# Sir-Teo/MuZero-Go

Hardware: AMD Instinct MI355X
Metric: MCTS simulations/sec (whole node) + self-play moves/sec, 9x9 Go, 200 sims/move (higher is better)
Workload: dtype fp32

## Files before the change

include/mzgo.h:

```cpp
#ifndef MZGO_H
#define MZGO_H

#include <stdint.h>

#ifdef __cplusplus
extern "C" {
#endif

enum {
  MZGO_OK = 0,
  MZGO_EINVAL = -1,
  MZGO_EHIP = -2,
  MZGO_ENOWEIGHTS = -3,
  MZGO_EASSERT = -4
};

typedef struct mzgo_config {
  int board_size;
  int latent_dim;
  int num_games;
  int num_simulations;
  int max_moves;
  int compat;
  int temperature_moves;
  int search_variant;
  double c_puct;
  double discount;
  double dirichlet_alpha;
  double dirichlet_epsilon;
  double pass_epsilon;
  double temperature;
  double komi;
  uint64_t seed;
  int game_base;
  int device;
  int direct_dynamics;
  int tower;
  int res_blocks;
  int fast_simulations;
  double full_search_prob;
} mzgo_config;

typedef struct mzgo_engine mzgo_engine;

void mzgo_default_config(mzgo_config* cfg, int board_size);

int mzgo_engine_create(const mzgo_config* cfg, mzgo_engine** out);
void mzgo_engine_destroy(mzgo_engine* eng);
int mzgo_playout_budget_host(uint64_t seed, uint32_t key_gid, int move, int num_simulations, int fast_simulations,
                             double full_search_prob, int* budget);
const char* mzgo_last_error(void);
int64_t mzgo_engine_device_bytes(const mzgo_engine* eng);

int mzgo_set_weights(mzgo_engine* eng, const char* key, const float* data_host,
                     const int64_t* shape, int ndim);
int mzgo_weights_ready(const mzgo_engine* eng);

int mzgo_set_weights_device(mzgo_engine* eng, const char* const* keys, const float* const* data_dev,
                            const int64_t* const* shapes, const int* ndims, int n, void* stream);
int mzgo_weights_copy(mzgo_engine* dst, const mzgo_engine* src, void* stream);
int mzgo_weights_export(mzgo_engine* eng, float* data_host, int64_t cap, int64_t* n_floats, void* stream);
int mzgo_weights_pack_host(int board_size, int latent_dim, const char* const* keys, const float* const* data_host,
                           const int64_t* const* shapes, const int* ndims, int n, float* blob, int64_t cap,
                           int64_t* n_floats);

int mzgo_initial_inference(mzgo_engine* eng, const float* obs, int B, float* latent,
                           float* value, float* logits, void* stream);
int mzgo_recurrent_inference(mzgo_engine* eng, const float* latent, const int64_t* action, int B,
                             float* next_latent, float* reward, float* value, float* logits,
                             void* stream);
int mzgo_check_inference_errors(mzgo_engine* eng, void* stream);

int mzgo_search(mzgo_engine* eng, const float* root_obs, const double* noise, int G, int move_index,
                int32_t* root_child_visits, double* root_value, void* stream);
int mzgo_reanalyse(mzgo_engine* eng, const int8_t* stones, const uint8_t* invd, const uint8_t* flags,
                   const int32_t* ids, const double* noise, int n, int32_t* visits, double* value,
                   double* policy, void* stream);
int mzgo_tree_export(mzgo_engine* eng, int g, int32_t* n_nodes_host, int32_t* child_host,
                     int32_t* visits_host, double* value_sum_host, float* prior_host,
                     double* root_prior_host, void* stream);

int mzgo_board_reset(mzgo_engine* eng, void* stream);
int mzgo_board_step(mzgo_engine* eng, const int32_t* actions, int32_t* status, double* winner,
                    void* stream);
int mzgo_board_planes(mzgo_engine* eng, double* planes, void* stream);
int mzgo_board_set(mzgo_engine* eng, int g, const int8_t* stones_host, const uint8_t* invd_host,
                   const int32_t* meta_host, void* stream);

int mzgo_selfplay_reset(mzgo_engine* eng, int epoch, void* stream);
int mzgo_selfplay_move(mzgo_engine* eng, void* stream);
int mzgo_selfplay_moves(mzgo_engine* eng, int moves, void* stream);

int mzgo_arena_move(mzgo_engine* eng, mzgo_engine* opponent, void* stream);
int mzgo_arena_moves(mzgo_engine* eng, mzgo_engine* opponent, int moves, void* stream);
int mzgo_selfplay_counters(mzgo_engine* eng, uint64_t* counters_host, void* stream);
int mzgo_search_stats(mzgo_engine* eng, uint64_t* stats_host, void* stream);
int mzgo_search_stats2(mzgo_engine* eng, uint64_t* stats_host, int cap, void* stream);

int mzgo_selfplay_set_timing(mzgo_engine* eng, int on);
int mzgo_selfplay_launch_times(mzgo_engine* eng, float* boards_ms, float* queue_ms, int cap, int* n_host);
int mzgo_stream_wait_started(mzgo_engine* eng, uint64_t target, void* stream);
int mzgo_tower_timing(mzgo_engine* eng, int enable, double* tower_ms_host, int64_t* towers_host);

int mzgo_dyn_conv_backward_workspace(int B, int C, int64_t* bytes_host);
int mzgo_dyn_conv_backward(const float* grad_out, const float* out, const float* latent, const int64_t* action,
                           const float* emb, const float* weight, int B, int C, int N, float* grad_latent,
                           float* grad_weight, float* grad_bias, void* workspace, int64_t workspace_bytes,
                           void* stream);
int mzgo_conv3x3_relu_forward(const float* x, const int64_t* action, const float* emb, const float* weight,
                              const float* bias, int B, int Cin, int Cout, int N, float* out, void* stream);
int mzgo_conv3x3_backward_workspace(int B, int Cin, int Cout, int64_t* bytes_host);
int mzgo_conv3x3_backward(const float* grad_out, const float* out, const float* x, const int64_t* action,
                          const float* emb, const float* weight, int B, int Cin, int Cout, int N, float* grad_x,
                          float* grad_weight, float* grad_bias, void* workspace, int64_t workspace_bytes,
                          void* stream);
int mzgo_selfplay_inject_noise(mzgo_engine* eng, const double* noise);
int mzgo_selfplay_record_noise(mzgo_engine* eng, double* dst);
// ... 199 lines not shown
```

muzero-go_amd/csrc/mzgo_board.hpp:

```cpp
#pragma once
#include "mzgo_common.hpp"

namespace mzgo {

struct BoardMeta {
  int turn;
  int passed;
  int done;
  int moves;
};

template <class G>
struct BoardLds {
  int8_t* stone;
  uint8_t* invd;
  int* label;
  int* libs;
  int* gsize;
  int* killed;
  int* misc;
};

template <class G>
struct BoardWG {
  static constexpr int SIZE = G::THREADS;
  __device__ static int id() { return tid_local(); }
  __device__ static void sync() { __syncthreads(); }
  __device__ static bool any(int v) { return __syncthreads_or(v) != 0; }
  __device__ static bool leader() { return tid_local() == 0; }
};
template <class G>
__device__ __forceinline__ bool nbr(int c, int d, int& n) {
  const int r = c / G::N, col = c - r * G::N;
  switch (d) {
    case 0: if (r == 0) return false; n = c - G::N; return true;
    case 1: if (r == G::N - 1) return false; n = c + G::N; return true;
    case 2: if (col == 0) return false; n = c - 1; return true;
    default: if (col == G::N - 1) return false; n = c + 1; return true;
  }
}

template <class G, class T, class ClassFn>
__device__ __forceinline__ void label_components(int* label, ClassFn cls) {
  for (int c = T::id(); c < G::CELLS; c += T::SIZE) label[c] = cls(c) ? c : -1;
  T::sync();
  for (int it = 0; it < G::CELLS + 2; ++it) {
    int changed = 0;
    for (int c = T::id(); c < G::CELLS; c += T::SIZE) {
      const int k = cls(c);
      if (!k) continue;
      int m = label[c];
#pragma unroll
      for (int d = 0; d < 4; ++d) {
// ... 9 lines not shown
}

template <class G, class T>
__device__ __forceinline__ void count_liberties(BoardLds<G>& b, bool sizes) {
  for (int c = T::id(); c < G::CELLS; c += T::SIZE) { b.libs[c] = 0; if (sizes) b.gsize[c] = 0; }
  T::sync();
  for (int c = T::id(); c < G::CELLS; c += T::SIZE) {
    if (b.stone[c]) {
      if (sizes) atomicAdd(&b.gsize[b.label[c]], 1);
      continue;
    }
    int seen[4];
    int ns = 0;
#pragma unroll
    for (int d = 0; d < 4; ++d) {
      int n;
      if (nbr<G>(c, d, n) && b.stone[n]) {
        int l = b.label[n];
        bool dup = false;
        for (int i = 0; i < ns; ++i) dup |= seen[i] == l;
        if (!dup) { seen[ns++] = l; atomicAdd(&b.libs[l], 1); }
      }
    }
  }
  T::sync();
}

template <class G, class T>
__device__ __forceinline__ void compute_invalid(BoardLds<G>& b, int mover, int ko) {
  for (int c = T::id(); c < G::CELLS; c += T::SIZE) {
    uint8_t inv;
    if (b.stone[c]) {
      inv = 1;
    } else {
      bool boxed = true, maybe_bad = false, surely_ok = false;
#pragma unroll
      for (int d = 0; d < 4; ++d) {
        int n;
        if (!nbr<G>(c, d, n)) continue;
        const int s = b.stone[n];
        if (!s) { boxed = false; continue; }
        const int lib = b.libs[b.label[n]];
        if (s - 1 == mover) { maybe_bad |= lib > 1; surely_ok |= lib == 1; }
        else                { maybe_bad |= lib == 1; surely_ok |= lib > 1; }
      }
      inv = (boxed && maybe_bad && !surely_ok) ? 1 : 0;
    }
    b.invd[c] = inv;
  }
  T::sync();
  if (ko >= 0 && T::leader()) b.invd[ko] = 1;
  T::sync();
}

enum : int { BOARD_OK = 0, BOARD_ERR_DONE = 1, BOARD_ERR_INVALID = 2, BOARD_ERR_RANGE = 3 };

template <class G, class T = BoardWG<G>>
__device__ __forceinline__ int board_step(BoardLds<G>& b, BoardMeta& m, int action) {
  if (m.done) return BOARD_ERR_DONE;
  if (action < 0 || action > G::CELLS) return BOARD_ERR_RANGE;
  const int player = m.turn;
  int ko = -1;
  if (action == G::CELLS) {
    if (m.passed) m.done = 1;
    m.passed = 1;
    label_components<G, T>(b.label, [&](int c) { return (int)b.stone[c]; });
    count_liberties<G, T>(b, false);
  } else {
    if (b.invd[action]) return BOARD_ERR_INVALID;
    m.passed = 0;
    if (T::leader()) {
      b.stone[action] = (int8_t)(player + 1);
      bool boxed = true;
      for (int d = 0; d < 4; ++d) {
        int n;
        if (nbr<G>(action, d, n)) boxed &= b.stone[n] == 2 - player;
      }
      b.misc[1] = boxed;
    }
    T::sync();
    label_components<G, T>(b.label, [&](int c) { return (int)b.stone[c]; });
    count_liberties<G, T>(b, true);
    if (T::leader()) {
      int nk = 0;
      for (int d = 0; d < 4; ++d) {
        int n;
        if (!nbr<G>(action, d, n) || b.stone[n] != 2 - player) continue;
        const int l = b.label[n];
        bool dup = false;
        for (int i = 0; i < nk; ++i) dup |= b.killed[i] == l;
        if (!dup && b.libs[l] == 0) b.killed[nk++] = l;
      }
      b.misc[0] = nk;
      b.misc[2] = (nk == 1 && b.misc[1] && b.gsize[b.killed[0]] == 1) ? b.killed[0] : -1;
    }
    T::sync();
    const int nk = b.misc[0];
    ko = b.misc[2];
    if (nk > 0) {
      for (int c = T::id(); c < G::CELLS; c += T::SIZE) {
        if (b.stone[c] == 2 - player) {
          const int l = b.label[c];
          bool dead = false;
          for (int i = 0; i < nk; ++i) dead |= b.killed[i] == l;
          if (dead) b.stone[c] = 0;
        }
      }
      T::sync();
// ... 47 lines not shown
```

muzero-go_amd/csrc/mzgo_kernels.hpp:

```cpp
#pragma once
#include "mzgo_jobs.hpp"
#include "mzgo_replay.hpp"

namespace mzgo {

template <class G>
constexpr bool rep_needs_scratch() {
  if constexpr (G::WINO) return Wino<G>::NSTRIP > 1;
  else return false;
}

struct NoRepJobs {
  __device__ bool operator()(int) const { return false; }
};

template <class G, class PlaneFn, class Jobs = NoRepJobs>
__device__ __forceinline__ void representation(Smem<G>& sm, const NetParams& np, PlaneFn planes, float* lat,
                                      int lat_stride, float* scr, unsigned long long* ts = nullptr,
                                      Jobs jobs = Jobs{}) {
  float* mid = rep_needs_scratch<G>() ? scr : lat;
  for (int i = tid_local(); i < 6 * G::CELLS; i += G::THREADS) {
    const int c = i / G::CELLS, j = i - c * G::CELLS;
    sm.u.in[c * G::CPAD + j] = planes(c, j);
  }
// ... 1411 lines not shown
      for (;;) {
        helper_loop<G>(sm, np_a_arg, np_b_arg, sp, E_arg, t);
        if (!sp.tail) break;
        t = join_running_game<G>(sm, E_arg, games, t);
        if (t < 0) break;
      }
    }
    return;
  }
  const int g = blockIdx.x;
  const EngineArrays& E = E_arg;
  if (tid_local() == 0) atomicAdd(&E_arg.counters[6], 1ull);
  auto release_helpers = [&]() {
    if ((sp.helpers > 0 || sp.tail) && tid_local() == 0) job_exit(job_of<G>(E_arg, g));
  };
  auto tail_phase = [&]() {
    if constexpr (Smem<G>::GLOBAL_Y && G::WINO) {
      if (sp.tail) {
        __syncthreads();
        for (int t = g; (t = join_running_game<G>(sm, E_arg, games, t)) >= 0;)
          helper_loop<G>(sm, np_a_arg, np_b_arg, sp, E_arg, t);
      }
    }
    if constexpr (TailConvs<G>::value)
      if (sp.tail) {
        __syncthreads();
#ifdef MZGO_STAMPS
        const unsigned long long th = __builtin_amdgcn_s_memtime();
#endif
        tail_help<G>(sm, np_a_arg, np_b_arg, E_arg, g, games);
#ifdef MZGO_STAMPS
        if (tid_local() == 0 && E_arg.stamps) E_arg.stamps[(size_t)blockIdx.x * kStampPhases + 47] +=
            __builtin_amdgcn_s_memtime() - th;
#endif
      }
  };
  if (E.status[g] != 0) { release_helpers(); tail_phase(); return; }
  if ((sp.helpers > 0 || sp.tail) && tid_local() == 0) job_mark_started(job_of<G>(E_arg, g));
  if constexpr (G::WINO) wino_raw_zero<G>(sm.raw);
  BoardMeta m;
  board_load<G>(sm.stone, sm.invd, E, g, m);
  for (int step = 0; step < pp.moves; ++step) {
    if (selfplay_one_move<G, CAPS>(sm, np_a_arg, np_b_arg, sp, pp, E_arg, g,
                             [&]() { return game_key_id(pp.game_base, g, pp.epoch); }, m))
      break;
    __syncthreads();
  }
  release_helpers();
  tail_phase();
}

template <class G>
struct BoardsGeo {
  static constexpr int THREADS = (G::CELLS + 63) / 64 * 64 < 512 ? (G::CELLS + 63) / 64 * 64 : 512;
};
template <class G>
struct BoardsTeam {
  static constexpr int SIZE = BoardsGeo<G>::THREADS;
  __device__ static int id() { return tid_local(); }
  __device__ static void sync() { __syncthreads(); }
  __device__ static bool any(int v) { return __syncthreads_or(v) != 0; }
  __device__ static bool leader() { return tid_local() == 0; }
};
template <class G>
struct BoardsSmem {
  TreeLds<G> t;
  int label[G::CELLS], libs[G::CELLS], gsize[G::CELLS];
  int8_t stone[G::CELLS];
  uint8_t invd[G::CELLS];
  int killed[4];
  int misc[8];
  int bc[8];
};

template <int N, int C, bool CAPS = false>
__global__ void __launch_bounds__((BoardsGeo<Geo<N, C>>::THREADS)) k_selfplay_boards(SearchParams sp, PlayParams pp,
                                                                                    EngineArrays E) {
  typedef Geo<N, C> G;
  typedef BoardsTeam<G> T;
  __shared__ BoardsSmem<G> sm;
  const int g = blockIdx.x;
  const int tid = tid_local();
  if (tid == 0) {
    atomicAdd(&E.counters[6], 1ull);
    E.mpq[2 * g + 1] = 0;
  }
  if (E.status[g] != 0) return;
  BoardMeta m;
  board_load<G, T>(sm.stone, sm.invd, E, g, m);
  BoardLds<G> b = make_board_lds<G>(sm.stone, sm.invd, sm.label, sm.libs, sm.gsize, sm.killed, sm.misc);
  const int mv_first = m.moves;
  int played = 0;
  const TreeView TV = TreeViewOf<G>::make(E, g);
  for (int step = 0; step < pp.moves; ++step) {
    const int mv = m.moves;
    const size_t rec = (size_t)g * E.max_moves + mv;
    const uint64_t key = move_key(sp, pp, g, mv);
    const int budget = move_budget<CAPS>(sp, key);
    record_observation<G, T>(E, rec, sm.stone, sm.invd, m, CAPS && budget != sp.num_simulations);
    ++played;
    build_mask<G, T>(sm.t, sp.pass_epsilon, [&](int a) { return sm.invd[a]; });
    if (wave_id() == 0) {
      const int a = choose_action<G>(sm.t, TV, sp.compat, move_temperature(pp, mv), key, E.rec_policy + rec * G::A);
      if (lane_id_local() == 0) {
        sm.bc[0] = a;
        E.rec_action[rec] = a;
      }
    }
    __syncthreads();
    double w;
    const int st = play_action<G, T>(E, g, b, m, sm.bc[0], pp.komi, w);
    if (finish_move<G, T>(E, budget, g, rec, st, m, w)) break;
    __syncthreads();
  }
  if (tid == 0) {
    E.mpq[2 * g] = mv_first;
    E.mpq[2 * g + 1] = played;
  }
}

template <int N, int C, bool CAPS = false>
__global__ void __launch_bounds__((Geo<N, C>::THREADS)) __attribute__((amdgpu_waves_per_eu(Geo<N, C>::WPE, Geo<N, C>::WPE))) k_search_queue(NetParams np_arg, SearchParams sp, PlayParams pp,
                                                            EngineArrays E_arg, int games) {
  typedef Geo<N, C> G;
  __shared__ Smem<G> sm;
  static_assert(sizeof(Smem<G>) <= 160 * 1024, "one workgroup per CU: the whole LDS at most");
  if constexpr (G::WINO) wino_raw_zero<G>(sm.raw);
  const int leaders = (int)gridDim.x - sp.helpers;
  if ((int)blockIdx.x >= leaders) {
    if constexpr (Smem<G>::GLOBAL_Y && G::WINO)
      helper_loop<G>(sm, np_arg, np_arg, sp, E_arg, ((int)blockIdx.x - leaders) % leaders);
    return;
  }
  const int slot = blockIdx.x;
  const int items = games * pp.moves;
  for (;;) {
    if (tid_local() == 0) sm.bc[0] = (int)atomicAdd((unsigned*)&E_arg.mpq[2 * games], 1u);
    __syncthreads();
    const int k = sm.bc[0];
    __syncthreads();
    if (k >= items) break;
    const int j = k / games, g = k % games;
    const int mv0 = __builtin_amdgcn_readfirstlane(E_arg.mpq[2 * g]);
    const int nmv = __builtin_amdgcn_readfirstlane(E_arg.mpq[2 * g + 1]);
    if (j >= nmv) continue;
    const int mv = mv0 + nmv - 1 - j;
    const EngineArrays E = launder_arrays(E_arg);
    const NetParams np = launder_params(np_arg);
    const size_t rec = (size_t)g * E.max_moves + mv;
    for (int c = tid_local(); c < G::CELLS; c += G::THREADS) {
      sm.stone[c] = E.rec_stones[rec * G::CELLS + c];
      sm.invd[c] = E.rec_invd[rec * G::CELLS + c];
    }
    const BoardMeta m0 = flags_unpack(E.rec_flags[rec], mv);
    __syncthreads();
    const uint64_t key = move_key(sp, pp, g, mv);
    const double* noise = pp.noise ? pp.noise + rec * G::A : nullptr;
    double* noise_out = pp.noise_out ? pp.noise_out + rec * G::A : nullptr;
    SearchParams spm = launder_search(sp);
    spm.net = 0;
    if constexpr (CAPS) spm.num_simulations = move_budget<CAPS>(sp, key);
    run_search<G>(sm, np, spm, E, slot, [&](int c, int jj) { return board_plane<G>(sm.stone, sm.invd, m0, c, jj); },
                  noise, key, nullptr, noise_out);
    if (tid_local() == 0) E.rec_value[rec] = root_value(TreeViewOf<G>::make(E, slot));
    __syncthreads();
  }
  if (sp.helpers > 0 && tid_local() == 0) job_exit(job_of<G>(E_arg, slot));
// ... 142 lines not shown
```

muzero-go_amd/csrc/mzgo_move.hpp:

```cpp
#pragma once
#include "mzgo_board.hpp"
#include "mzgo_search.hpp"

namespace mzgo {

constexpr int kCounters = 14;

struct EngineArrays {
  int S;
  int max_moves;
  float* pool;
  float* prior;
  int* child;
  int* visits;
  double* wsum;
  double* root_prior;
  int* path;
  int* nodes;
  int* nact;
  double* cval;
  int8_t* stones;
  uint8_t* invd;
  int* meta;
  int8_t* rec_stones;
// ... 185 lines not shown
    if (compat == 1) { const int c = T.child[a]; v = c >= 0 ? (double)T.visits[c] : 0.0; }
    t.dbuf[a] = v * mask_of<G>(t, a);
  }
  wave_lds_sync();
  const double vsum = np_pairwise_sum<double, G::A>(t.dbuf);
#pragma unroll
  for (int j = 0; j < G::AP; ++j) { const int a = lane + 64 * j; vc[j] = a < G::A ? t.dbuf[a] : 0.0; }
  wave_lds_sync();
  for (int a = lane; a < G::A; a += 64) t.dbuf[a] = mask_of<G>(t, a);
  wave_lds_sync();
  msum = np_pairwise_sum<double, G::A>(t.dbuf);
#pragma unroll
  for (int j = 0; j < G::AP; ++j) {
    const int a = lane + 64 * j;
    if (a < G::A) pol[a] = vsum > 0 ? vc[j] / vsum : mask_of<G>(t, a) / msum;
  }
  return vsum;
}

template <class G>
__device__ __forceinline__ int choose_action_main(TreeLds<G>& t, const TreeView& T, uint64_t key, double* pol) {
  const int lane = lane_id_local();
  double vc[G::AP], msum;
  const double tot = visit_policy<G>(t, T, 1, 1, pol, vc, msum);
  if (tot > 0) return argmax_action<G>(vc);
  const int action = pick_valid<G>(t, draw(key, TAG_ACTION, 0));
#pragma unroll
  for (int j = 0; j < G::AP; ++j) {
    const int a = lane + 64 * j;
    if (a < G::A) pol[a] = a == action ? 1.0 : 0.0;
  }
  return action;
}

template <class G>
__device__ __forceinline__ int choose_action(TreeLds<G>& t, const TreeView& T, int compat, double temperature,
                                    uint64_t key, double* pol) {
  const int lane = lane_id_local();
  double vcm[G::AP], msum;
  const double vsum = visit_policy<G>(t, T, 0, compat, pol, vcm, msum);
  const uint64_t h = draw(key, TAG_ACTION, 0);
  if (temperature == 0.0) return vsum > 0 ? argmax_action<G>(vcm) : pick_valid<G>(t, h);
  const double e = 1.0 / temperature;
#pragma unroll
  for (int j = 0; j < G::AP; ++j) {
    const int a = lane + 64 * j;
    if (a < G::A) t.dbuf[a] = (e == 1.0 ? vcm[j] : pow(vcm[j], e)) * mask_of<G>(t, a);
  }
  wave_lds_sync();
  const double ts = np_pairwise_sum<double, G::A>(t.dbuf);
  wave_lds_sync();
  for (int a = lane; a < G::A; a += 64) t.dbuf[a] = ts > 0 ? t.dbuf[a] / ts : mask_of<G>(t, a) / msum;
  wave_lds_sync();
  if (lane == 0) {
    double cdf = 0.0;
    for (int a = 0; a < G::A; ++a) cdf += t.dbuf[a];
    const double total = cdf;
    const double u = u01(h);
    double run = 0.0;
    int idx = 0;
    for (int a = 0; a < G::A; ++a) {
      run += t.dbuf[a];
      if (run / total <= u) idx = a + 1;
    }
    t.bcast = idx;
  }
  wave_lds_sync();
  return t.bcast;
}

__device__ __forceinline__ double move_temperature(const PlayParams& pp, int mv) {
  return mv < pp.temperature_moves ? pp.temperature : 0.0;
}
template <class G>
__device__ __forceinline__ int choose_move_action(TreeLds<G>& t, const TreeView& T, const SearchParams& sp,
                                                  const PlayParams& pp, int mv, uint64_t key, double* pol) {
  return sp.variant == 1 ? choose_action_main<G>(t, T, key, pol)
                         : choose_action<G>(t, T, sp.compat, move_temperature(pp, mv), key, pol);
}

__device__ __forceinline__ double root_value(const TreeView& T) {
  const int n = T.visits[0];
  return n > 0 ? T.wsum[0] / (double)n : 0.0;
}

template <class G, class T = BoardWG<G>>
__device__ __forceinline__ int play_action(const EngineArrays& E, int g, BoardLds<G>& b, BoardMeta& m, int action,
                                           double komi, double& w) {
  const int st = board_step<G, T>(b, m, action);
  T::sync();
  w = (st == BOARD_OK && m.done) ? board_winning<G, T>(b, komi) : 0.0;
  board_store<G, T>(b.stone, b.invd, E, g, m);
  return st;
}

template <class G, class T = BoardWG<G>>
__device__ __forceinline__ bool finish_move(const EngineArrays& E, int sims, int g, size_t rec, int st,
                                            const BoardMeta& m, double w) {
  const bool ended = m.done || m.moves >= E.max_moves;
  if (T::leader()) {
    E.rec_reward[rec] = w;
    atomicAdd(&E.counters[0], (unsigned long long)sims);
    atomicAdd(&E.counters[1], 1ull);
    if (st != BOARD_OK) {
      E.status[g] = 16 + st;
    } else if (ended) {
      E.status[g] = 1;
      E.game_len[g] = m.moves;
      E.final_reward[g] = m.done ? w : 0.0;
      atomicAdd(&E.counters[2], 1ull);
    }
  }
  return st != BOARD_OK || ended;
}

}
```

muzero-go_amd/mzgo/__init__.py:

```python
from ._lib import MzgoError
from .arena import SelfPlayEvaluator
from .engine import Engine, EngineConfig, pack_weights_host, playout_budget_host
from .env import GoEnv
from .loss import unroll_loss, unroll_loss_host
from .net import MuZeroNet
from .optim import DeviceAdam, adam_step_host, optim_chunk
from .ownership import OwnershipHead, ownership_loss, ownership_loss_host
from .reanalyse import Reanalyser, positions_from_planes, record_ids
from .replay import (DeviceReplay, ownership_host, ownership_targets_host, position_priorities_host, queue_key_gids,
                     sample_positions_host, value_targets_host, window_items_host)
from .resnet import ResMuZeroNet
from .search import MCTS, MainMCTS, MuZeroAgent
from .selfplay import GameHistory, SelfPlay, history_from_device, save_batches
from .unroll import bf16_round_host, unroll, unroll_heads_host
from .weights import deterministic_res_state_dict, deterministic_state_dict

__all__ = ["Engine", "EngineConfig", "GoEnv", "MuZeroNet", "MCTS", "MainMCTS", "MuZeroAgent", "SelfPlay",
           "GameHistory", "history_from_device", "save_batches", "deterministic_state_dict", "SelfPlayEvaluator",
           "ResMuZeroNet", "deterministic_res_state_dict", "MzgoError", "Reanalyser",
           "positions_from_planes", "record_ids", "DeviceReplay", "queue_key_gids", "unroll_loss",
           "unroll_loss_host", "unroll", "unroll_heads_host", "bf16_round_host", "window_items_host", "value_targets_host",
           "sample_positions_host", "position_priorities_host", "DeviceAdam", "adam_step_host", "optim_chunk",
           "playout_budget_host", "OwnershipHead", "ownership_loss", "ownership_loss_host", "ownership_host",
           "ownership_targets_host", "pack_weights_host"]
```

muzero-go_amd/mzgo/_lib.py:

```python
import ctypes
import os

import torch

LIB_PATH = os.environ.get("MZGO_LIB") or os.path.join(os.path.dirname(os.path.abspath(__file__)), "libmzgo.so")

MZGO_OK, MZGO_EINVAL, MZGO_EHIP, MZGO_ENOWEIGHTS, MZGO_EASSERT = 0, -1, -2, -3, -4


class Config(ctypes.Structure):

    _fields_ = [
        ("board_size", ctypes.c_int),
        ("latent_dim", ctypes.c_int),
        ("num_games", ctypes.c_int),
        ("num_simulations", ctypes.c_int),
        ("max_moves", ctypes.c_int),
        ("compat", ctypes.c_int),
        ("temperature_moves", ctypes.c_int),
        ("search_variant", ctypes.c_int),
        ("c_puct", ctypes.c_double),
        ("discount", ctypes.c_double),
        ("dirichlet_alpha", ctypes.c_double),
        ("dirichlet_epsilon", ctypes.c_double),
        ("pass_epsilon", ctypes.c_double),
        ("temperature", ctypes.c_double),
        ("komi", ctypes.c_double),
        ("seed", ctypes.c_uint64),
        ("game_base", ctypes.c_int),
        ("device", ctypes.c_int),
        ("direct_dynamics", ctypes.c_int),
        ("tower", ctypes.c_int),
        ("res_blocks", ctypes.c_int),
        ("fast_simulations", ctypes.c_int),
        ("full_search_prob", ctypes.c_double),
    ]


class OptimHyper(ctypes.Structure):

    _fields_ = [
        ("lr0", ctypes.c_double),
        ("beta1", ctypes.c_double),
        ("beta2", ctypes.c_double),
        ("eps", ctypes.c_double),
        ("weight_decay", ctypes.c_double),
        ("decoupled", ctypes.c_int),
        ("max_norm", ctypes.c_double),
        ("step_size", ctypes.c_int64),
        ("gamma", ctypes.c_double),
    ]


_P = ctypes.c_void_p
_I = ctypes.c_int
_L = ctypes.c_int64
SIGNATURES = {
    "mzgo_default_config": (None, [ctypes.POINTER(Config), _I]),
    "mzgo_engine_create": (_I, [ctypes.POINTER(Config), ctypes.POINTER(_P)]),
    "mzgo_engine_destroy": (None, [_P]),
    "mzgo_playout_budget_host": (_I, [ctypes.c_uint64, ctypes.c_uint32, _I, _I, _I, ctypes.c_double,
                                      ctypes.POINTER(_I)]),
    "mzgo_last_error": (ctypes.c_char_p, []),
    "mzgo_engine_device_bytes": (ctypes.c_int64, [_P]),
    "mzgo_set_weights": (_I, [_P, ctypes.c_char_p, _P, ctypes.POINTER(ctypes.c_int64), _I]),
    "mzgo_weights_ready": (_I, [_P]),
    "mzgo_set_weights_device": (_I, [_P, _P, _P, _P, _P, _I, _P]),
    "mzgo_weights_copy": (_I, [_P, _P, _P]),
    "mzgo_weights_export": (_I, [_P, _P, ctypes.c_int64, ctypes.POINTER(ctypes.c_int64), _P]),
    "mzgo_weights_pack_host": (_I, [_I, _I, _P, _P, _P, _P, _I, _P, ctypes.c_int64, ctypes.POINTER(ctypes.c_int64)]),
    "mzgo_initial_inference": (_I, [_P, _P, _I, _P, _P, _P, _P]),
    "mzgo_recurrent_inference": (_I, [_P, _P, _P, _I, _P, _P, _P, _P, _P]),
    "mzgo_check_inference_errors": (_I, [_P, _P]),
    "mzgo_search": (_I, [_P, _P, _P, _I, _I, _P, _P, _P]),
    "mzgo_reanalyse": (_I, [_P, _P, _P, _P, _P, _P, _I, _P, _P, _P, _P]),
    "mzgo_tree_export": (_I, [_P, _I, _P, _P, _P, _P, _P, _P, _P]),
    "mzgo_board_reset": (_I, [_P, _P]),
    "mzgo_board_step": (_I, [_P, _P, _P, _P, _P]),
    "mzgo_board_planes": (_I, [_P, _P, _P]),
    "mzgo_board_set": (_I, [_P, _I, _P, _P, _P, _P]),
    "mzgo_selfplay_reset": (_I, [_P, _I, _P]),
    "mzgo_selfplay_move": (_I, [_P, _P]),
    "mzgo_selfplay_moves": (_I, [_P, _I, _P]),
    "mzgo_arena_move": (_I, [_P, _P, _P]),
    "mzgo_arena_moves": (_I, [_P, _P, _I, _P]),
    "mzgo_selfplay_counters": (_I, [_P, _P, _P]),
    "mzgo_search_stats": (_I, [_P, _P, _P]),
    "mzgo_search_stats2": (_I, [_P, _P, _I, _P]),
    "mzgo_selfplay_set_timing": (_I, [_P, _I]),
    "mzgo_selfplay_launch_times": (_I, [_P, _P, _P, _I, _P]),
    "mzgo_stream_wait_started": (_I, [_P, ctypes.c_uint64, _P]),
    "mzgo_tower_timing": (_I, [_P, _I, _P, _P]),
    "mzgo_selfplay_inject_noise": (_I, [_P, _P]),
    "mzgo_selfplay_record_noise": (_I, [_P, _P]),
    "mzgo_tower_record_nodes": (_I, [_P, _P]),
    "mzgo_records_export": (_I, [_P, _I, _P, _P, _P, _P, _P, _P, _P, _P, _P, _P, _P]),
    "mzgo_records_pack": (_I, [_P, _P, ctypes.c_int64, _P, _P]),
    "mzgo_dyn_conv_backward_workspace": (_I, [_I, _I, ctypes.POINTER(ctypes.c_int64)]),
    "mzgo_dyn_conv_backward": (_I, [_P, _P, _P, _P, _P, _P, _I, _I, _I, _P, _P, _P, _P, ctypes.c_int64, _P]),
    "mzgo_conv3x3_relu_forward": (_I, [_P, _P, _P, _P, _P, _I, _I, _I, _I, _P, _P]),
    "mzgo_conv3x3_backward_workspace": (_I, [_I, _I, _I, ctypes.POINTER(ctypes.c_int64)]),
    "mzgo_conv3x3_backward": (_I, [_P, _P, _P, _P, _P, _P, _I, _I, _I, _I, _P, _P, _P, _P, ctypes.c_int64, _P]),
    "mzgo_replay_create": (_I, [_I, _I, _I, _I, ctypes.POINTER(_P)]),
    "mzgo_replay_destroy": (None, [_P]),
    "mzgo_replay_info": (_I, [_P, _P, _P, _P, _P]),
    "mzgo_replay_add_games": (_I, [_P, _P, _P]),
    "mzgo_replay_play_games": (_I, [_P, _P, _I, _I, _P]),
    "mzgo_replay_add": (_I, [_P, _I, _P, _P, _P, _P, _P, _P, _P, ctypes.c_int32, _P]),
    "mzgo_replay_export": (_I, [_P, _I, _P, _P, _P, _P, _P, _P, _P, _P, _P, _P]),
    "mzgo_replay_batch": (_I, [_P, _P, _P, _P, _I, _I, ctypes.c_double, _P, _P, _P, _P, _P, _P, _P, _P, _P]),
    "mzgo_replay_finish_values": (_I, [_P, _P, _P, _P, _I, _P, _P]),
    "mzgo_replay_reanalyse": (_I, [_P, _P, _P, _I, _P]),
    "mzgo_replay_symmetry_table": (_I, [_I, _I, _P, _P]),
    "mzgo_replay_sample": (_I, [_P, _I, ctypes.c_uint64, ctypes.c_uint32, _I, ctypes.c_double, _P, _P, _P, _P, _P]),
    "mzgo_replay_sample_batch": (_I, [_P, _I, _I, ctypes.c_double, ctypes.c_uint64, ctypes.c_uint32, _I,
                                      ctypes.c_double] + [_P] * 13),
    "mzgo_replay_batch_items": (_I, [_P, _P, _I, _I, ctypes.c_double] + [_P] * 9),
    "mzgo_replay_reanalyse_sample": (_I, [_P, _P, _P, _I, _I, _P, _P]),
    "mzgo_replay_window_items_host": (_I, [_P, _I, _P, _I, _I, _P, _P]),
    "mzgo_replay_batch_values": (_I, [_P, _P, _P, _P, _I, _I, _I, ctypes.c_double] + [_P] * 6),
    "mzgo_replay_batch_items_values": (_I, [_P, _P, _I, _I, _I, ctypes.c_double] + [_P] * 6),
    "mzgo_replay_sample_batch_values": (_I, [_P, _I, _I, _I, ctypes.c_double, ctypes.c_uint64, ctypes.c_uint32, _I,
                                             ctypes.c_double] + [_P] * 10),
# ... 108 lines not shown
```

muzero-go_amd/mzgo/engine.py:

```python
import ctypes
from dataclasses import dataclass, fields

import numpy as np
import torch

from . import _lib
from ._lib import check, lib, ptr, stream_of


@dataclass
class EngineConfig:

    board_size: int = 9
    latent_dim: int = 96
    num_games: int = 1
    num_simulations: int = 128
    max_moves: int = 0
    compat: str = "reference"
    temperature_moves: int = 15
    search_variant: str = "self_play"
    c_puct: float = 2.5
    discount: float = 0.99
    dirichlet_alpha: float = 0.15
    dirichlet_epsilon: float = 0.02
# ... 22 lines not shown
                if v not in ("self_play", "main"):
                    raise ValueError(f"search_variant must be 'self_play' or 'main', not {v!r}")
                v = 0 if v == "self_play" else 1
            if f.name == "dynamics":
                if v not in ("factored", "direct"):
                    raise ValueError(f"dynamics must be 'factored' or 'direct', not {v!r}")
                c.direct_dynamics = 0 if v == "factored" else 1
                continue
            setattr(c, f.name, v)
        return c


def playout_budget_host(seed, key_gid, move, num_simulations, fast_simulations, full_search_prob):
    out = ctypes.c_int()
    check(lib.mzgo_playout_budget_host(int(seed), int(key_gid) & 0xFFFFFFFF, int(move), int(num_simulations),
                                       int(fast_simulations), float(full_search_prob), ctypes.byref(out)))
    return out.value


def _weight_table(items, A):
    items = list(items)
    n = len(items)
    keys = (ctypes.c_char_p * n)()
    data = (ctypes.c_void_p * n)()
    shapes = (ctypes.POINTER(ctypes.c_int64) * n)()
    ndims = (ctypes.c_int * n)()
    keep = []
    for i, (key, t) in enumerate(items):
        a = np.ascontiguousarray(torch.as_tensor(t).detach().to("cpu", torch.float32).numpy())
        if key == "dynamics.action_embedding.weight" and a.ndim == 2 and a.shape[0] > A:
            a = np.ascontiguousarray(a[:A])
        shape = (ctypes.c_int64 * max(a.ndim, 1))(*a.shape)
        keep.append((a, shape))
        keys[i] = key.encode()
        data[i] = a.ctypes.data
        shapes[i] = ctypes.cast(shape, ctypes.POINTER(ctypes.c_int64))
        ndims[i] = a.ndim
    return keys, data, shapes, ndims, n, keep


def pack_weights_host(state_dict, board_size):
    items = list(state_dict.items() if hasattr(state_dict, "items") else state_dict)
    N = int(board_size)
    widths = [np.shape(t)[-1] for k, t in items if k == "dynamics.action_embedding.weight" and np.ndim(t) == 2]
    if not widths:
        raise _lib.MzgoError("mzgo error -1: missing weight 'dynamics.action_embedding.weight'")
    keys, data, shapes, ndims, n, keep = _weight_table(items, N * N + 1)
    total = ctypes.c_int64()
    check(lib.mzgo_weights_pack_host(N, int(widths[0]), keys, data, shapes, ndims, n, None, 0, ctypes.byref(total)))
    out = np.empty(total.value, np.float32)
    check(lib.mzgo_weights_pack_host(N, int(widths[0]), keys, data, shapes, ndims, n, ptr(out), out.size,
                                     ctypes.byref(total)))
    return out


class Engine:
    def __init__(self, config: EngineConfig):
        self.config = config
        self.N = config.board_size
        self.C = config.latent_dim
        self.A = self.N * self.N + 1
        self.G = config.num_games
        self.S = config.num_simulations
        self.M = config.max_moves or self.N * self.N
        self.device = torch.device("cuda", config.device)
        if not torch.cuda.is_available():
            raise RuntimeError("mzgo needs a ROCm GPU (MI355X); no CPU fallback exists")
        torch.cuda.init()
        h = ctypes.c_void_p()
        check(lib.mzgo_engine_create(ctypes.byref(config.to_c()), ctypes.byref(h)))
        self._h = h
        self._weights_key = None

    def close(self):
        if getattr(self, "_h", None):
            lib.mzgo_engine_destroy(self._h)
            self._h = None

    def __del__(self):
        try:
            self.close()
        except Exception:
            pass

    @property
    def handle(self):
        return self._h

    def device_bytes(self):
        return int(lib.mzgo_engine_device_bytes(self._h))

    def set_state_dict(self, state_dict):
        for key, t in state_dict.items():
            a = np.ascontiguousarray(torch.as_tensor(t).detach().to("cpu", torch.float32).numpy())
            if key == "dynamics.action_embedding.weight" and a.ndim == 2 and a.shape[0] > self.A:
                a = np.ascontiguousarray(a[:self.A])
            shape = (ctypes.c_int64 * a.ndim)(*a.shape)
            check(lib.mzgo_set_weights(self._h, key.encode(), ptr(a), shape, a.ndim))
        if not lib.mzgo_weights_ready(self._h):
            check(_lib.MZGO_ENOWEIGHTS)

    def set_parameters_device(self, named_tensors):
        items = list(named_tensors.items() if hasattr(named_tensors, "items") else named_tensors)
        n = len(items)
        keys = (ctypes.c_char_p * n)()
        data = (ctypes.c_void_p * n)()
# ... 206 lines not shown
```

Measured before the change: 142.8 million.

## Replace LDS label-propagation board with single-wave bitboard Go engine in self-play kernel

Introduces a bitboard Go representation where each of 64 lanes holds its group's mask, using dilation and ballots for captures, liberties and illegal moves. The self-play kernel drops to 64 threads and one wave, which removes LDS label propagation, atomics and block-wide barriers per move. Action sampling now builds a wave-parallel CDF with lane reads and a ballot instead of a serial lane-0 loop. It also adds a host-side bitboard play API for testing, and the shrunken block size may change occupancy and latency of other per-move phases.

```diff
diff --git a/include/mzgo.h b/include/mzgo.h
--- a/include/mzgo.h
+++ b/include/mzgo.h
@@ -63,6 +63,10 @@
 int mzgo_weights_pack_host(int board_size, int latent_dim, const char* const* keys, const float* const* data_host,
                            const int64_t* const* shapes, const int* ndims, int n, float* blob, int64_t cap,
                            int64_t* n_floats);
+
+int mzgo_boards_host_play(int board_size, const int8_t* stones, const uint8_t* invd, const int32_t* meta,
+                          const int32_t* actions, int n_actions, double komi, int8_t* out_stones,
+                          uint8_t* out_invd, int32_t* out_meta, int32_t* out_status, double* out_winner);
 
 int mzgo_initial_inference(mzgo_engine* eng, const float* obs, int B, float* latent,
                            float* value, float* logits, void* stream);
diff --git a/muzero-go_amd/csrc/mzgo_bitboard.hip b/muzero-go_amd/csrc/mzgo_bitboard.hip
--- /dev/null
+++ b/muzero-go_amd/csrc/mzgo_bitboard.hip
@@ -0,0 +1,71 @@
+#include <hip/hip_runtime.h>
+
+#include <vector>
+
+#include "../../include/mzgo.h"
+#include "mzgo_bitboard.hpp"
+
+namespace mzgo {
+int set_error(int code, const char* fmt, ...);
+
+namespace {
+
+template <int N>
+void host_play(const int8_t* stones, const uint8_t* invd, const int32_t* meta, const int32_t* actions, int n,
+               double komi, int8_t* out_stones, uint8_t* out_invd, int32_t* out_meta, int32_t* out_status,
+               double* out_winner) {
+  constexpr int CELLS = N * N;
+  std::vector<int8_t> st0(CELLS, 0);
+  std::vector<uint8_t> iv0(CELLS, 0);
+  if (stones) st0.assign(stones, stones + CELLS);
+  if (invd) iv0.assign(invd, invd + CELLS);
+  bb::State<N> s;
+  bb::HostTeam<N> team;
+  bb::init_from_board<N>(s, team, st0.data(), iv0.data(), meta ? meta[0] : 0, meta ? meta[1] : 0, meta ? meta[2] : 0,
+                         meta ? meta[3] : 0);
+  for (int i = 0; i < n; ++i) {
+    const int status = bb::step<N>(s, team, actions[i]);
+    if (out_status) out_status[i] = status;
+    if (out_winner) out_winner[i] = (status == BOARD_OK && s.done) ? bb::winning<N>(s, komi) : 0.0;
+    if (out_meta) {
+      int32_t* mm = out_meta + (size_t)i * 4;
+      mm[0] = s.turn; mm[1] = s.passed; mm[2] = s.done; mm[3] = s.moves;
+    }
+    for (int lane = 0; lane < 64; ++lane)
+      bb::lane_planes<N>(s, lane, [&](int c, int8_t sv, uint8_t iv) {
+        if (out_stones) out_stones[(size_t)i * CELLS + c] = sv;
+        if (out_invd) out_invd[(size_t)i * CELLS + c] = iv;
+      });
+  }
+}
+
+}
+}
+
+using namespace mzgo;
+
+extern "C" int mzgo_boards_host_play(int board_size, const int8_t* stones, const uint8_t* invd, const int32_t* meta,
+                                     const int32_t* actions, int n_actions, double komi, int8_t* out_stones,
+                                     uint8_t* out_invd, int32_t* out_meta, int32_t* out_status, double* out_winner) {
+  const char* fn = "mzgo_boards_host_play";
+  if (n_actions < 0) return set_error(MZGO_EINVAL, "%s: n_actions must be >= 0, got %d", fn, n_actions);
+  if (n_actions > 0 && !actions) return set_error(MZGO_EINVAL, "%s: null actions", fn);
+  if (stones)
+    for (int c = 0; c < board_size * board_size && board_size > 0 && board_size <= 19; ++c)
+      if (stones[c] < 0 || stones[c] > 2)
+        return set_error(MZGO_EINVAL, "%s: stones[%d] = %d (0 empty, 1 black, 2 white)", fn, c, (int)stones[c]);
+  switch (board_size) {
+#define MZGO_PLAY(N)                                                                                            \
+  case N:                                                                                                       \
+    host_play<N>(stones, invd, meta, actions, n_actions, komi, out_stones, out_invd, out_meta, out_status,      \
+                 out_winner);                                                                                   \
+    return MZGO_OK;
+    MZGO_PLAY(5)
+    MZGO_PLAY(6)
+    MZGO_PLAY(9)
+    MZGO_PLAY(19)
+#undef MZGO_PLAY
+    default:
+      return set_error(MZGO_EINVAL, "%s: no kernels built for board_size %d", fn, board_size);
+  }
+}
diff --git a/muzero-go_amd/csrc/mzgo_bitboard.hpp b/muzero-go_amd/csrc/mzgo_bitboard.hpp
--- /dev/null
+++ b/muzero-go_amd/csrc/mzgo_bitboard.hpp
@@ -0,0 +1,346 @@
+#pragma once
+#include <hip/hip_runtime.h>
+#include <stdint.h>
+
+#define MZGO_HD __host__ __device__ __forceinline__
+
+namespace mzgo {
+
+enum : int { BOARD_OK = 0, BOARD_ERR_DONE = 1, BOARD_ERR_INVALID = 2, BOARD_ERR_RANGE = 3 };
+
+namespace bb {
+
+template <int W>
+struct Bits {
+  uint64_t v[W];
+
+  MZGO_HD static constexpr Bits zero() {
+    Bits r{};
+    for (int w = 0; w < W; ++w) r.v[w] = 0;
+    return r;
+  }
+  MZGO_HD static Bits bit(int c) {
+    Bits r{};
+#pragma unroll
+    for (int w = 0; w < W; ++w) r.v[w] = (c >> 6) == w ? 1ull << (c & 63) : 0ull;
+    return r;
+  }
+  MZGO_HD constexpr Bits operator|(const Bits& o) const {
+    Bits r{};
+    for (int w = 0; w < W; ++w) r.v[w] = v[w] | o.v[w];
+    return r;
+  }
+  MZGO_HD constexpr Bits operator&(const Bits& o) const {
+    Bits r{};
+    for (int w = 0; w < W; ++w) r.v[w] = v[w] & o.v[w];
+    return r;
+  }
+  MZGO_HD constexpr Bits operator~() const {
+    Bits r{};
+    for (int w = 0; w < W; ++w) r.v[w] = ~v[w];
+    return r;
+  }
+  MZGO_HD bool operator==(const Bits& o) const {
+    uint64_t d = 0;
+#pragma unroll
+    for (int w = 0; w < W; ++w) d |= v[w] ^ o.v[w];
+    return d == 0;
+  }
+  MZGO_HD bool any() const {
+    uint64_t d = 0;
+#pragma unroll
+    for (int w = 0; w < W; ++w) d |= v[w];
+    return d != 0;
+  }
+  MZGO_HD int count() const {
+    int n = 0;
+#pragma unroll
+    for (int w = 0; w < W; ++w) n += __builtin_popcountll(v[w]);
+    return n;
+  }
+  MZGO_HD int first() const {
+    int c = 0;
+    bool found = false;
+#pragma unroll
+    for (int w = 0; w < W; ++w)
+      if (!found && v[w]) { c = 64 * w + __builtin_ctzll(v[w]); found = true; }
+    return c;
+  }
+  MZGO_HD bool test(int c) const {
+    uint64_t x = 0;
+#pragma unroll
+    for (int w = 0; w < W; ++w) x = (c >> 6) == w ? v[w] : x;
+    return (x >> (c & 63)) & 1;
+  }
+  MZGO_HD bool test(int q, int lane) const { return (v[q] >> lane) & 1; }
+  template <int K>
+  MZGO_HD Bits shl() const {
+    Bits r{};
+#pragma unroll
+    for (int w = 0; w < W; ++w) r.v[w] = (v[w] << K) | (w > 0 ? v[w > 0 ? w - 1 : 0] >> (64 - K) : 0ull);
+    return r;
+  }
+  template <int K>
+  MZGO_HD Bits shr() const {
+    Bits r{};
+#pragma unroll
+    for (int w = 0; w < W; ++w) r.v[w] = (v[w] >> K) | (w + 1 < W ? v[w + 1 < W ? w + 1 : w] << (64 - K) : 0ull);
+    return r;
+  }
+};
+template <int W>
+MZGO_HD Bits<W> select(bool c, const Bits<W>& a, const Bits<W>& b) {
+  Bits<W> r{};
+#pragma unroll
+  for (int w = 0; w < W; ++w) r.v[w] = c ? a.v[w] : b.v[w];
+  return r;
+}
+
+template <int N>
+struct Board {
+  static_assert(N >= 2 && N <= 19, "board sizes 2..19");
+  static constexpr int CELLS = N * N;
+  static constexpr int W = (CELLS + 63) / 64;
+  typedef Bits<W> B;
+
+  MZGO_HD static constexpr B full() {
+    B r{};
+    for (int w = 0; w < W; ++w) {
+      const int n = CELLS - 64 * w;
+      r.v[w] = n >= 64 ? ~0ull : (1ull << n) - 1;
+    }
+    return r;
+  }
+  MZGO_HD static constexpr B column(int col) {
+    B r = B::zero();
+    for (int row = 0; row < N; ++row) {
+      const int c = row * N + col;
+      r.v[c >> 6] |= 1ull << (c & 63);
+    }
+    return r;
+  }
+  MZGO_HD static B dil(const B& x) {
+    constexpr B not_last = full() & ~column(N - 1), not_first = full() & ~column(0), all = full();
+    const B r = (x & not_last).template shl<1>() | (x & not_first).template shr<1>() |
+                x.template shl<N>() | x.template shr<N>();
+    return r & all;
+  }
+  MZGO_HD static int nbr(int c, int d) {
+    const int r = c / N, col = c - r * N;
+    switch (d) {
+      case 0: return r == 0 ? -1 : c - N;
+      case 1: return r == N - 1 ? -1 : c + N;
+      case 2: return col == 0 ? -1 : c - 1;
+      default: return col == N - 1 ? -1 : c + 1;
+    }
+  }
+};
+
+template <int N>
+struct State {
+  typename Board<N>::B st[2];
+  typename Board<N>::B inv;
+  int turn, passed, done, moves;
+};
+
+template <int N, class Team>
+MZGO_HD void init_from_board(State<N>& s, Team& t, const int8_t* stone, const uint8_t* invd, int turn, int passed,
+                             int done, int moves) {
+  typedef Board<N> Bd;
+  typedef typename Bd::B B;
+  s.turn = turn; s.passed = passed; s.done = done; s.moves = moves;
+#pragma unroll
+  for (int q = 0; q < Bd::W; ++q) {
+    uint64_t b0, b1, i0, i1;
+    t.ballot2([&](int lane, B*) {
+      const int c = lane + 64 * q;
+      return c < Bd::CELLS ? (int)stone[c] : 0;
+    }, b0, b1);
+    t.ballot2([&](int lane, B*) {
+      const int c = lane + 64 * q;
+      return c < Bd::CELLS && invd[c] ? 1 : 0;
+    }, i0, i1);
+    s.st[0].v[q] = b0; s.st[1].v[q] = b1; s.inv.v[q] = i0;
+  }
+  const B st0 = s.st[0], st1 = s.st[1];
+  t.each([&](int lane, B* g) {
+#pragma unroll
+    for (int q = 0; q < Bd::W; ++q)
+      g[q] = (st0.test(q, lane) || st1.test(q, lane)) ? B::bit(lane + 64 * q) : B::zero();
+  });
+  for (int it = 0; it < Bd::CELLS; ++it) {
+    uint64_t ch, unused;
+    t.ballot2([&](int lane, B* g) {
+      int changed = 0;
+#pragma unroll
+      for (int q = 0; q < Bd::W; ++q) {
+        const B grown = (g[q] | Bd::dil(g[q])) & select(st0.test(q, lane), st0, st1);
+        changed |= !(grown == g[q]);
+        g[q] = grown;
+      }
+      return changed;
+    }, ch, unused);
+    if (!ch) break;
+  }
+}
+
+template <int N, class Team>
+MZGO_HD int step(State<N>& s, Team& t, int action) {
+  typedef Board<N> Bd;
+  typedef typename Bd::B B;
+  if (s.done) return BOARD_ERR_DONE;
+  if (action < 0 || action > Bd::CELLS) return BOARD_ERR_RANGE;
+  const bool p = s.turn != 0;
+  constexpr B all = Bd::full();
+  B own = select(p, s.st[1], s.st[0]), opp = select(p, s.st[0], s.st[1]);
+  int ko = -1;
+  if (action == Bd::CELLS) {
+    if (s.passed) s.done = 1;
+    s.passed = 1;
+  } else {
+    if (s.inv.test(action)) return BOARD_ERR_INVALID;
+    s.passed = 0;
+    const B a = B::bit(action);
+    const bool boxed = !(Bd::dil(a) & ~opp).any();
+    own = own | a;
+    B merged = a;
+#pragma unroll
+    for (int d = 0; d < 4; ++d) {
+      const int n = Bd::nbr(action, d);
+      if (n >= 0 && own.test(n)) merged = merged | t.fetch(n);
+    }
+    t.each([&](int lane, B* g) {
+#pragma unroll
+      for (int q = 0; q < Bd::W; ++q) g[q] = select(merged.test(q, lane), merged, g[q]);
+    });
+    const B emp = all & ~(own | opp);
+    B captured = B::zero();
+    int nk = 0;
+#pragma unroll
+    for (int d = 0; d < 4; ++d) {
+      const int n = Bd::nbr(action, d);
+      if (n >= 0 && opp.test(n)) {
+        const B k = t.fetch(n);
+        if (!(k & captured).any() && !(Bd::dil(k) & emp).any()) { captured = captured | k; ++nk; }
+      }
+    }
+    if (nk > 0) {
+      if (nk == 1 && boxed && captured.count() == 1) ko = captured.first();
+      opp = opp & ~captured;
+      t.each([&](int lane, B* g) {
+#pragma unroll
+        for (int q = 0; q < Bd::W; ++q) g[q] = select(captured.test(q, lane), B::zero(), g[q]);
+      });
+    }
+  }
+  const B occ = own | opp, emp = all & ~occ;
+  B atari, many;
+#pragma unroll
+  for (int q = 0; q < Bd::W; ++q) {
+    t.ballot2([&](int lane, B* g) {
+      const int l = g[q].any() ? (Bd::dil(g[q]) & emp).count() : 0;
+      return l == 1 ? 1 : (l > 1 ? 2 : 0);
+    }, atari.v[q], many.v[q]);
+  }
+  const B maybe_bad = (many & own) | (atari & opp), surely_ok = (atari & own) | (many & opp);
+  B inv = occ | (emp & ~Bd::dil(emp) & Bd::dil(maybe_bad) & ~Bd::dil(surely_ok));
+  if (ko >= 0) inv = inv | B::bit(ko);
+  s.inv = inv;
+  s.st[0] = select(p, opp, own);
+  s.st[1] = select(p, own, opp);
+  s.turn = p ? 0 : 1;
+  s.moves += 1;
+  return BOARD_OK;
+}
+
+template <int N>
+MZGO_HD double winning(const State<N>& s, double komi) {
+  typedef Board<N> Bd;
+  typedef typename Bd::B B;
+  constexpr B all = Bd::full();
+  const B emp = all & ~(s.st[0] | s.st[1]);
+  B reach[2];
+#pragma unroll
+  for (int col = 0; col < 2; ++col) {
+    B f = Bd::dil(s.st[col]) & emp;
+    for (int it = 0; it < Bd::CELLS; ++it) {
+      const B n = (f | Bd::dil(f)) & emp;
+      if (n == f) break;
+      f = n;
+    }
+    reach[col] = f;
+  }
+  const int black = (s.st[0] | (reach[0] & ~reach[1])).count();
+  const int white = (s.st[1] | (reach[1] & ~reach[0])).count();
+  const double diff = (double)black - (double)white - komi;
+  return diff > 0 ? 1.0 : (diff < 0 ? -1.0 : 0.0);
+}
+
+template <int N, class F>
+MZGO_HD void lane_planes(const State<N>& s, int lane, F put) {
+  typedef Board<N> Bd;
+#pragma unroll
+  for (int q = 0; q < Bd::W; ++q) {
+    const int c = lane + 64 * q;
+    if (c < Bd::CELLS)
+      put(c, (int8_t)(s.st[0].test(q, lane) ? 1 : (s.st[1].test(q, lane) ? 2 : 0)), (uint8_t)s.inv.test(q, lane));
+  }
+}
+
+template <int N>
+struct HostTeam {
+  typedef typename Board<N>::B B;
+  B g[64][Board<N>::W];
+  B fetch(int c) const { return g[c & 63][c >> 6]; }
+  template <class F>
+  void each(F f) {
+    for (int lane = 0; lane < 64; ++lane) f(lane, g[lane]);
+  }
+  template <class F>
+  void ballot2(F f, uint64_t& b0, uint64_t& b1) {
+    b0 = b1 = 0;
+    for (int lane = 0; lane < 64; ++lane) {
+      const int k = f(lane, g[lane]);
+      b0 |= (uint64_t)(k & 1) << lane;
+      b1 |= (uint64_t)((k >> 1) & 1) << lane;
+    }
+  }
+};
+
+#if defined(__HIPCC__)
+template <int N>
+struct WaveTeam {
+  typedef typename Board<N>::B B;
+  static constexpr int W = Board<N>::W;
+  B g[W];
+  __device__ __forceinline__ static int lane() { return (int)(threadIdx.x & 63u); }
+  __device__ __forceinline__ B fetch(int c) const {
+    c = __builtin_amdgcn_readfirstlane(c);
+    const int q = c >> 6, l = c & 63;
+    B r = B::zero();
+#pragma unroll
+    for (int qq = 0; qq < W; ++qq) {
+      if (qq == q) {
+#pragma unroll
+        for (int w = 0; w < W; ++w) {
+          const uint32_t lo = (uint32_t)__builtin_amdgcn_readlane((int)(uint32_t)g[qq].v[w], l);
+          const uint32_t hi = (uint32_t)__builtin_amdgcn_readlane((int)(uint32_t)(g[qq].v[w] >> 32), l);
+          r.v[w] = (uint64_t)lo | ((uint64_t)hi << 32);
+        }
+      }
+    }
+    return r;
+  }
+  template <class F>
+  __device__ __forceinline__ void each(F f) { f(lane(), g); }
+  template <class F>
+  __device__ __forceinline__ void ballot2(F f, uint64_t& b0, uint64_t& b1) {
+    const int k = f(lane(), g);
+    b0 = __ballot(k & 1);
+    b1 = __ballot(k & 2);
+  }
+};
+#endif
+
+}
+}
diff --git a/muzero-go_amd/csrc/mzgo_board.hpp b/muzero-go_amd/csrc/mzgo_board.hpp
--- a/muzero-go_amd/csrc/mzgo_board.hpp
+++ b/muzero-go_amd/csrc/mzgo_board.hpp
@@ -1,4 +1,5 @@
 #pragma once
+#include "mzgo_bitboard.hpp"
 #include "mzgo_common.hpp"
 
 namespace mzgo {
@@ -114,8 +115,6 @@
   if (ko >= 0 && T::leader()) b.invd[ko] = 1;
   T::sync();
 }
-
-enum : int { BOARD_OK = 0, BOARD_ERR_DONE = 1, BOARD_ERR_INVALID = 2, BOARD_ERR_RANGE = 3 };
 
 template <class G, class T = BoardWG<G>>
 __device__ __forceinline__ int board_step(BoardLds<G>& b, BoardMeta& m, int action) {
diff --git a/muzero-go_amd/csrc/mzgo_kernels.hpp b/muzero-go_amd/csrc/mzgo_kernels.hpp
--- a/muzero-go_amd/csrc/mzgo_kernels.hpp
+++ b/muzero-go_amd/csrc/mzgo_kernels.hpp
@@ -1487,7 +1487,7 @@
 
 template <class G>
 struct BoardsGeo {
-  static constexpr int THREADS = (G::CELLS + 63) / 64 * 64 < 512 ? (G::CELLS + 63) / 64 * 64 : 512;
+  static constexpr int THREADS = 64;
 };
 template <class G>
 struct BoardsTeam {
@@ -1500,12 +1500,8 @@
 template <class G>
 struct BoardsSmem {
   TreeLds<G> t;
-  int label[G::CELLS], libs[G::CELLS], gsize[G::CELLS];
   int8_t stone[G::CELLS];
   uint8_t invd[G::CELLS];
-  int killed[4];
-  int misc[8];
-  int bc[8];
 };
 
 template <int N, int C, bool CAPS = false>
@@ -1523,10 +1519,22 @@
   if (E.status[g] != 0) return;
   BoardMeta m;
   board_load<G, T>(sm.stone, sm.invd, E, g, m);
-  BoardLds<G> b = make_board_lds<G>(sm.stone, sm.invd, sm.label, sm.libs, sm.gsize, sm.killed, sm.misc);
+  bb::State<N> s;
+  bb::WaveTeam<N> team;
+  bb::init_from_board<N>(s, team, sm.stone, sm.invd, m.turn, m.passed, m.done, m.moves);
   const int mv_first = m.moves;
   int played = 0;
   const TreeView TV = TreeViewOf<G>::make(E, g);
+#ifdef MZGO_STAMPS
+  unsigned long long tl[4] = {0, 0, 0, 0}, tl0 = __builtin_amdgcn_s_memtime();
+  auto lap = [&](int k) {
+    const unsigned long long now = __builtin_amdgcn_s_memtime();
+    tl[k] += now - tl0;
+    tl0 = now;
+  };
+#else
+  auto lap = [](int) {};
+#endif
   for (int step = 0; step < pp.moves; ++step) {
     const int mv = m.moves;
     const size_t rec = (size_t)g * E.max_moves + mv;
@@ -1535,19 +1543,36 @@
     record_observation<G, T>(E, rec, sm.stone, sm.invd, m, CAPS && budget != sp.num_simulations);
     ++played;
     build_mask<G, T>(sm.t, sp.pass_epsilon, [&](int a) { return sm.invd[a]; });
-    if (wave_id() == 0) {
-      const int a = choose_action<G>(sm.t, TV, sp.compat, move_temperature(pp, mv), key, E.rec_policy + rec * G::A);
-      if (lane_id_local() == 0) {
-        sm.bc[0] = a;
-        E.rec_action[rec] = a;
-      }
-    }
-    __syncthreads();
-    double w;
-    const int st = play_action<G, T>(E, g, b, m, sm.bc[0], pp.komi, w);
-    if (finish_move<G, T>(E, budget, g, rec, st, m, w)) break;
-    __syncthreads();
-  }
+    lap(0);
+    const int a = __builtin_amdgcn_readfirstlane(
+        choose_action<G>(sm.t, TV, sp.compat, move_temperature(pp, mv), key, E.rec_policy + rec * G::A));
+    if (tid == 0) E.rec_action[rec] = a;
+    lap(1);
+    const int st = bb::step<N>(s, team, a);
+    lap(2);
+    double w = 0.0;
+    if (st == BOARD_OK) {
+      bb::lane_planes<N>(s, bb::WaveTeam<N>::lane(), [&](int c, int8_t sv, uint8_t iv) {
+        sm.stone[c] = sv;
+        sm.invd[c] = iv;
+      });
+      m = BoardMeta{s.turn, s.passed, s.done, s.moves};
+      if (m.done) w = bb::winning<N>(s, pp.komi);
+    }
+    const bool over = finish_move<G, T>(E, budget, g, rec, st, m, w);
+    lap(3);
+    if (over) break;
+    __syncthreads();
+  }
+  __syncthreads();
+  board_store<G, T>(sm.stone, sm.invd, E, g, m);
+#ifdef MZGO_STAMPS
+  if (tid == 0 && E.stamps) {
+    unsigned long long* sl = E.stamps + (size_t)blockIdx.x * kStampPhases;
+    for (int k = 0; k < 4; ++k) sl[83 + k] += tl[k];
+    sl[87] += tl[1] + tl[2] + tl[3];
+  }
+#endif
   if (tid == 0) {
     E.mpq[2 * g] = mv_first;
     E.mpq[2 * g + 1] = played;
diff --git a/muzero-go_amd/csrc/mzgo_move.hpp b/muzero-go_amd/csrc/mzgo_move.hpp
--- a/muzero-go_amd/csrc/mzgo_move.hpp
+++ b/muzero-go_amd/csrc/mzgo_move.hpp
@@ -261,21 +261,33 @@
   wave_lds_sync();
   for (int a = lane; a < G::A; a += 64) t.dbuf[a] = ts > 0 ? t.dbuf[a] / ts : mask_of<G>(t, a) / msum;
   wave_lds_sync();
-  if (lane == 0) {
-    double cdf = 0.0;
-    for (int a = 0; a < G::A; ++a) cdf += t.dbuf[a];
-    const double total = cdf;
-    const double u = u01(h);
-    double run = 0.0;
-    int idx = 0;
-    for (int a = 0; a < G::A; ++a) {
-      run += t.dbuf[a];
-      if (run / total <= u) idx = a + 1;
-    }
-    t.bcast = idx;
-  }
-  wave_lds_sync();
-  return t.bcast;
+  double pr[G::AP], cdf[G::AP];
+#pragma unroll
+  for (int j = 0; j < G::AP; ++j) {
+    const int a = lane + 64 * j;
+    pr[j] = a < G::A ? t.dbuf[a] : 0.0;
+    cdf[j] = 0.0;
+  }
+  double run = 0.0;
+#pragma unroll
+  for (int j = 0; j < G::AP; ++j) {
+    const int n = G::A - 64 * j < 64 ? G::A - 64 * j : 64;
+    for (int l = 0; l < n; ++l) {
+      run += dpp::lane(pr[j], l);
+      cdf[j] = lane == l ? run : cdf[j];
+    }
+  }
+  const double total = run;
+  const double u = u01(h);
+  int idx = 0;
+#pragma unroll
+  for (int j = 0; j < G::AP; ++j) {
+    const int a = lane + 64 * j;
+    const uint64_t le = __ballot(a < G::A && cdf[j] / total <= u);
+    if (le) idx = 64 * j + 64 - __builtin_clzll(le);
+  }
+  wave_lds_sync();
+  return idx;
 }
 
 __device__ __forceinline__ double move_temperature(const PlayParams& pp, int mv) {
diff --git a/muzero-go_amd/mzgo/__init__.py b/muzero-go_amd/mzgo/__init__.py
--- a/muzero-go_amd/mzgo/__init__.py
+++ b/muzero-go_amd/mzgo/__init__.py
@@ -1,6 +1,6 @@
 from ._lib import MzgoError
 from .arena import SelfPlayEvaluator
-from .engine import Engine, EngineConfig, pack_weights_host, playout_budget_host
+from .engine import Engine, EngineConfig, boards_host_play, pack_weights_host, playout_budget_host
 from .env import GoEnv
 from .loss import unroll_loss, unroll_loss_host
 from .net import MuZeroNet
@@ -22,4 +22,4 @@
            "unroll_loss_host", "unroll", "unroll_heads_host", "bf16_round_host", "window_items_host", "value_targets_host",
            "sample_positions_host", "position_priorities_host", "DeviceAdam", "adam_step_host", "optim_chunk",
            "playout_budget_host", "OwnershipHead", "ownership_loss", "ownership_loss_host", "ownership_host",
-           "ownership_targets_host", "pack_weights_host"]
+           "ownership_targets_host", "pack_weights_host", "boards_host_play"]
diff --git a/muzero-go_amd/mzgo/_lib.py b/muzero-go_amd/mzgo/_lib.py
--- a/muzero-go_amd/mzgo/_lib.py
+++ b/muzero-go_amd/mzgo/_lib.py
@@ -69,6 +69,7 @@
     "mzgo_weights_copy": (_I, [_P, _P, _P]),
     "mzgo_weights_export": (_I, [_P, _P, ctypes.c_int64, ctypes.POINTER(ctypes.c_int64), _P]),
     "mzgo_weights_pack_host": (_I, [_I, _I, _P, _P, _P, _P, _I, _P, ctypes.c_int64, ctypes.POINTER(ctypes.c_int64)]),
+    "mzgo_boards_host_play": (_I, [_I, _P, _P, _P, _P, _I, ctypes.c_double, _P, _P, _P, _P, _P]),
     "mzgo_initial_inference": (_I, [_P, _P, _I, _P, _P, _P, _P]),
     "mzgo_recurrent_inference": (_I, [_P, _P, _P, _I, _P, _P, _P, _P, _P]),
     "mzgo_check_inference_errors": (_I, [_P, _P]),
diff --git a/muzero-go_amd/mzgo/engine.py b/muzero-go_amd/mzgo/engine.py
--- a/muzero-go_amd/mzgo/engine.py
+++ b/muzero-go_amd/mzgo/engine.py
@@ -98,6 +98,33 @@
     check(lib.mzgo_weights_pack_host(N, int(widths[0]), keys, data, shapes, ndims, n, ptr(out), out.size,
                                      ctypes.byref(total)))
     return out
+
+
+def boards_host_play(board_size, actions, state=None, komi=0.0):
+    N = int(board_size)
+    acts = np.ascontiguousarray(np.asarray(actions, dtype=np.int32).reshape(-1))
+    n = acts.size
+    stones = invd = meta = None
+    if state is not None:
+        st = np.asarray(state, dtype=np.float64).reshape(6, N * N)
+        stones = np.ascontiguousarray((st[0] > 0) * 1 + (st[1] > 0) * 2, dtype=np.int8)
+        invd = np.ascontiguousarray(st[3] > 0, dtype=np.uint8)
+        meta = np.array([st[2].max() > 0, st[4].max() > 0, st[5].max() > 0, 0], dtype=np.int32)
+    out_stones = np.zeros((n, N * N), np.int8)
+    out_invd = np.zeros((n, N * N), np.uint8)
+    out_meta = np.zeros((n, 4), np.int32)
+    status = np.zeros(n, np.int32)
+    winner = np.zeros(n, np.float64)
+    check(lib.mzgo_boards_host_play(N, ptr(stones), ptr(invd), ptr(meta), ptr(acts), n, float(komi), ptr(out_stones),
+                                    ptr(out_invd), ptr(out_meta), ptr(status), ptr(winner)))
+    planes = np.zeros((n, 6, N * N), np.float64)
+    planes[:, 0] = out_stones == 1
+    planes[:, 1] = out_stones == 2
+    planes[:, 2] = out_meta[:, 0:1]
+    planes[:, 3] = out_invd
+    planes[:, 4] = out_meta[:, 1:2]
+    planes[:, 5] = out_meta[:, 2:3]
+    return planes.reshape(n, 6, N, N), status, winner
 
 
 class Engine:
```

New measurement: 144.1 million, median of 6. No clear change (+1.0%).
